# Apokleos/kata-xpu-device-plugin

Measured on NVIDIA H100. Metric: pci.ids parse GB/s (x1000 text + 2^20-key join); device lookups/s reported beside it, higher is better.
Workload: dtype u8

## Files before the change

### kata-xpu-device-plugin_b200/csrc/api.cu

```cuda
#include <algorithm>
#include <cstdlib>
#include <new>
#include <vector>

#include "internal.cuh"
#include "pciids5.cu"
#include "finalize.cuh"
#include "small.cuh"
#include "scan.cuh"

void kx_exchange_destroy(kxpu_ctx *ctx);

static const char *kx_err_names[] = {
    "ok", "invalid argument", "CUDA error", "no sm_90 GPU available", "output buffer too small",
    "table capacity exceeded", "NCCL / peer exchange unavailable or failed", "input outside the supported domain", "out of memory"};

extern "C" const char *kxpu_strerror(int32_t status) {
    int i = -status;
    if (i < 0 || i > 8) return "unknown status";
    return kx_err_names[i];
}

extern "C" const char *kxpu_last_error(kxpu_ctx *ctx) {
    if (!ctx) return "null ctx";
// ... 175 lines not shown
        KX_SET_ERR(ctx, "cudaMalloc(%zu) for the look-back state failed", want * 8);
        return nullptr;
    }
    if (ctx->scan_state) cudaFree(ctx->scan_state);
    ctx->scan_state = p;
    ctx->scan_state_words = want;
    return p;
}

uint32_t kx_next_epoch(kxpu_ctx *ctx) {
    if (++ctx->scan_epoch >= ctx->scan_epoch_limit) {
        if (ctx->scan_state) cudaMemsetAsync(ctx->scan_state, 0, ctx->scan_state_words * 8, ctx->stream);
        ctx->scan_epoch = 1;
    }
    return ctx->scan_epoch;
}

static inline size_t align_up(size_t x, size_t a) { return (x + a - 1) / a * a; }

static inline size_t range_words_bytes(uint32_t num_chunks) { return ((size_t)num_chunks + 64) * 24; }

struct ArenaLayout {
    size_t o_slots, o_vfirst, o_trunc, ff_bytes, o_counters, o_range, o_row_key, o_row_line, o_row_anchor, o_row_noff, o_row_nlen,
        o_sel, o_blob, total;
};
static ArenaLayout arena_layout(uint32_t cap, uint32_t blob_cap, size_t range_bytes) {
    ArenaLayout L;
    const size_t slots = (size_t)cap + 1;
    size_t off = 0;
    L.o_slots = off;       off = align_up(off + slots * sizeof(KxSlot), 256);
    L.o_vfirst = off;      off = align_up(off + 65536 * 8, 256);
    L.o_trunc = off;       off = align_up(off + 8, 256);
    L.ff_bytes = off;
    L.o_counters = off;    off = align_up(off + KX_C_COUNT * 4, 256);
    L.o_range = off;       off = align_up(off + range_bytes, 256);
    L.o_row_key = off;     off = align_up(off + slots * 4, 256);
    L.o_row_line = off;    off = align_up(off + slots * 8, 256);
    L.o_row_anchor = off;  off = align_up(off + slots * 8, 256);
    L.o_row_noff = off;    off = align_up(off + slots * 4, 256);
    L.o_row_nlen = off;    off = align_up(off + slots * 4, 256);
    L.o_sel = off;         off = align_up(off + slots * 4, 256);
    L.o_blob = off;        off = align_up(off + (size_t)blob_cap + 16, 256);
    L.total = off;
    return L;
}

static void arena_reset(kxpu_ctx *ctx, const KxArena &a) {
    const ArenaLayout L = arena_layout(a.cap, a.blob_cap, a.range_bytes);
    const size_t n16 = L.ff_bytes / 16;
    size_t blocks = (n16 + 255) / 256;
    const size_t maxb = (size_t)ctx->sm_count * 8;
    if (blocks > maxb) blocks = maxb;
    kxparse::arena_reset_kernel<<<(unsigned)blocks, 256, 0, ctx->stream>>>((uint4 *)a.p, n16, (uint32_t *)((uint8_t *)a.p + L.o_counters));
    KX_LAUNCHED(ctx);
}

int32_t kx_table_acquire(kxpu_ctx *ctx, uint32_t cap, uint32_t blob_cap, uint32_t num_chunks, kxpu_table **out) {
    kxpu_table *t = new (std::nothrow) kxpu_table();
    if (!t) return KXPU_E_NOMEM;
    const size_t need_range = range_words_bytes(num_chunks);
    bool found = false;
    for (size_t i = 0; i < ctx->pool.size(); i++) {
        const KxArena &a = ctx->pool[i];
        if (a.cap == cap && a.blob_cap == blob_cap && a.range_bytes >= need_range && a.range_bytes <= 4 * need_range + (1u << 20)) {
// ... 22 lines not shown
        }
        arena_reset(ctx, a);
        t->arena = a;
    }
    const ArenaLayout L = arena_layout(cap, blob_cap, t->arena.range_bytes);
    uint8_t *b = (uint8_t *)t->arena.p;
    t->cap = cap;
    uint32_t lg = 0;
    while ((1u << lg) < cap) lg++;
    t->shift = 32 - lg;
    t->dev.slots = (KxSlot *)(b + L.o_slots);
    t->dev.vendor_first = (unsigned long long *)(b + L.o_vfirst);
    t->dev.trunc = (unsigned long long *)(b + L.o_trunc);
    t->dev.counters = (uint32_t *)(b + L.o_counters);
    t->dev.cap = cap;
    t->dev.shift = t->shift;
    t->dev.max_keys = cap / 2;
    t->range_words = (unsigned long long *)(b + L.o_range);
    t->row_key = (uint32_t *)(b + L.o_row_key);
    t->row_line = (unsigned long long *)(b + L.o_row_line);
    t->row_anchor = (unsigned long long *)(b + L.o_row_anchor);
    t->row_name_off = (uint32_t *)(b + L.o_row_noff);
    t->row_name_len = (uint32_t *)(b + L.o_row_nlen);
    t->sel = (uint32_t *)(b + L.o_sel);
    t->blob = b + L.o_blob;
    t->blob_cap = blob_cap;
    t->rows_cap = cap + 1;
    *out = t;
    return KXPU_OK;
}

void kx_table_release(kxpu_ctx *ctx, kxpu_table *t) {
    if (!t) return;
    if (t->arena.p) {
        if (ctx->pool.size() >= 4) {
            cudaStreamSynchronize(ctx->stream);
            cudaFree(ctx->pool.front().p);
            ctx->pool.erase(ctx->pool.begin());
        }
        arena_reset(ctx, t->arena);
        ctx->pool.push_back(t->arena);
    }
    delete t;
}

uint32_t kx_initial_blob_cap(kxpu_ctx *ctx, size_t n) {
    const uint32_t by_text = (uint32_t)std::min<size_t>(std::max<size_t>(n, 256), 4u << 20);
// ... 83 lines not shown
    if (wait) F.wait = *wait;
    F.text = d_text; F.n = n; F.base = base; F.tab = t->dev;
    if (mv) F.mv = *mv;
    else { F.mv.a = t->dev.vendor_first; F.mv.stride = 0; F.mv.n = 1; F.mv.trunc1 = t->dev.trunc; }
    F.row_key = t->row_key; F.row_line = t->row_line; F.row_anchor = t->row_anchor;
    F.row_name_off = t->row_name_off; F.row_name_len = t->row_name_len;
    F.blob = t->blob; F.blob_cap = t->blob_cap;
    if (slab) {
        F.slab_rows = reinterpret_cast<kxx::SlabRow *>(slab->rows); F.slab_rows_cap = slab->rows_cap;
        F.blob = slab->blob; F.blob_cap = slab->blob_cap;
        F.tail = slab->tail;
    }
    KxTimer tm(ctx, KXPU_T_FINALIZE);
    F.scan_w = t->cap >= (1u << 19) ? 32u : 8u;
    if (ctx->force_scan_w) F.scan_w = (uint32_t)ctx->force_scan_w;
    const unsigned batches = (t->cap + 1 + F.scan_w - 1) / F.scan_w;
    const unsigned grid = std::min<unsigned>((batches + kxparse::SF_WARPS - 1) / kxparse::SF_WARPS, 8u * ctx->sm_count);
    kxparse::select_finalize_kernel<<<grid, kxparse::SF_WARPS * 32, 0, ctx->stream>>>(F);
    KX_LAUNCHED(ctx);
    KX_CUDA(ctx, cudaGetLastError());
    return KXPU_OK;
}

int32_t kx_launch_lookup(kxpu_ctx *ctx, kxpu_table *t, const uint32_t *d_keys, size_t n, int32_t *d_rows) {
    if (n == 0) return KXPU_OK;
    KxTimer tm(ctx, KXPU_T_LOOKUP);
    size_t blocks = (n + 255) / 256;
    size_t maxb = (size_t)ctx->sm_count * 32;
    if (blocks > maxb) blocks = maxb;
    kxparse::lookup_kernel<<<(unsigned)blocks, 256, 0, ctx->stream>>>(d_keys, n, t->dev.slots, t->cap, t->shift, d_rows);
    KX_LAUNCHED(ctx);
    KX_CUDA(ctx, cudaGetLastError());
    return KXPU_OK;
}

struct KxJoin {
    const uint32_t *d_keys;
    size_t n;
    int32_t *d_rows;
    int32_t *h_rows;
    const uint8_t *src_text;
};

static void *kx_mapped_host(const void *p) {
    if (!p) return nullptr;
    cudaPointerAttributes at;
    if (cudaPointerGetAttributes(&at, p) != cudaSuccess) { cudaGetLastError(); return nullptr; }
    return at.type == cudaMemoryTypeHost ? at.devicePointer : nullptr;
}

static uint32_t small_text_chunks(kxpu_ctx *ctx) {
    if (ctx->small_chunks < 0) {
        int coop = 0, per_sm = 0;
// ... 89 lines not shown

static int32_t kx_build_table_join(kxpu_ctx *ctx, const uint8_t *d_text, size_t n, kxpu_table **out, const KxJoin *join) {
    if ((reinterpret_cast<uintptr_t>(d_text) & 15u) != 0) {
        KX_SET_ERR(ctx, "device text pointer must be 16-byte aligned");
        return KXPU_E_INVALID;
    }
    if (n >= (1ull << 44)) return KXPU_E_UNSUPPORTED;
    uint32_t cap = ctx->cap_hint;
    while (cap > (1u << 16) && (size_t)cap / 2 > n / 6 + 1) cap >>= 1;
    uint32_t blob_cap = kx_initial_blob_cap(ctx, n);
    const uint32_t num_chunks = (uint32_t)((n + kxparse::CW - 1) / kxparse::CW);
    bool have_trunc = false;
    for (int attempt = 0; attempt < 12; attempt++) {
        kxpu_table *t = nullptr;
        int32_t rc = kx_table_acquire(ctx, cap, blob_cap, num_chunks, &t);
        if (rc != KXPU_OK) return rc;
        const bool small_path = num_chunks > 0 && num_chunks <= small_text_chunks(ctx) && !have_trunc;
        if (small_path) {
            rc = launch_small(ctx, t, d_text, n, join);
        } else {
            if (join && join->src_text && attempt == 0) cudaMemcpyAsync(const_cast<uint8_t *>(d_text), join->src_text, n, cudaMemcpyDefault, ctx->stream);
            rc = kx_launch_parse(ctx, t, d_text, n, 0, 0, nullptr);
            if (rc == KXPU_OK && have_trunc) rc = kx_launch_trunc(ctx, t, d_text, n, 0);
            if (rc == KXPU_OK) rc = kx_launch_finalize(ctx, t, d_text, n, 0, nullptr, nullptr, nullptr);
            if (rc == KXPU_OK && join) rc = kx_launch_lookup(ctx, t, join->d_keys, join->n, join->d_rows);
        }
        if (rc != KXPU_OK) { kx_table_release(ctx, t); return rc; }
        const bool zero_copy = small_path && join && join->src_text;
        if (!zero_copy) {
            if (join && join->h_rows && join->n) cudaMemcpyAsync(join->h_rows, join->d_rows, join->n * 4, cudaMemcpyDeviceToHost, ctx->stream);
            cudaMemcpyAsync(ctx->h_ctl, t->dev.counters, KX_C_COUNT * 4, cudaMemcpyDeviceToHost, ctx->stream);
        }
        cudaError_t e = cudaStreamSynchronize(ctx->stream);
        if (e != cudaSuccess) {
            KX_SET_ERR(ctx, "parse/finalize failed: %s", cudaGetErrorString(e));
            kx_table_release(ctx, t);
            return KXPU_E_CUDA;
        }
        const uint32_t *h = ctx->h_ctl;
        if (h[KX_C_OVERFLOW] || h[KX_C_NKEYS] > t->dev.max_keys) {
            kx_table_release(ctx, t);
            if (!kx_grow_cap(&cap, h[KX_C_OVERFLOW] != 0)) return KXPU_E_CAPACITY;
            continue;
        }
        if (h[KX_C_NEED_TRUNC] == 2u) {
            kx_table_release(ctx, t);
            have_trunc = true;
            continue;
// ... 203 lines not shown
```

### kata-xpu-device-plugin_b200/csrc/finalize.cuh

```cuda
#pragma once
#include "exchange.cuh"
#include "parse_common.cuh"

namespace kxparse {

constexpr unsigned long long MAX_TOKEN = 65536ull;

__global__ void __launch_bounds__(1024) trunc_kernel(const uint8_t *__restrict__ text, unsigned long long n,
                                                      unsigned long long base, unsigned long long *trunc_out, uint32_t *counters) {
    __shared__ unsigned long long s_first[1024], s_last[1024], s_bad[1024];
    const unsigned long long per = (n + 1023ull) / 1024ull;
    const unsigned long long lo = per * threadIdx.x, hi = lo + per < n ? lo + per : n;
    unsigned long long first = KX_NO_OFF, last = KX_NO_OFF, bad = KX_NO_OFF;
    for (unsigned long long i = lo; i < hi; i++) {
        if (text[i] == (uint8_t)'\n') {
            if (first == KX_NO_OFF) first = i;
            else if (i - last - 1 >= MAX_TOKEN && bad == KX_NO_OFF) bad = last + 1;
            last = i;
        }
    }
    s_first[threadIdx.x] = first; s_last[threadIdx.x] = last; s_bad[threadIdx.x] = bad;
    __syncthreads();
    if (threadIdx.x == 0) {
        unsigned long long prev_nl = KX_NO_OFF;
// ... 83 lines not shown
__device__ __forceinline__ void finalize_store_row(const FinalizeParams &F, uint32_t row, uint32_t slot, uint32_t key, unsigned long long line,
                                                   unsigned long long anchor, uint32_t name_off, uint32_t name_len) {
    F.tab.slots[slot].row = (int32_t)row;
    if (F.slab_rows) {
        if (row < F.slab_rows_cap) {
            kxx::SlabRow r;
            r.key = key; r.name_len = name_len; r.line = line; r.anchor = anchor; r.name_off = name_off; r.pad = 0u;
            F.slab_rows[row] = r;
        }
    } else {
        F.row_key[row] = key; F.row_line[row] = line; F.row_anchor[row] = anchor;
        F.row_name_off[row] = name_off; F.row_name_len[row] = name_len;
    }
}

struct SfEntry {
    unsigned long long line, anchor;
    uint32_t slot, key;
};
constexpr int SF_QCAP = SF_BATCH - 1 + 32;

#define SF_MARK(k) do { if (F.trace && threadIdx.x == 0 && F.trace[blockIdx.x * 8u + (k)] == 0) F.trace[blockIdx.x * 8u + (k)] = clock64(); } while (0)

__device__ __forceinline__ void select_finalize_body(const FinalizeParams &F, const uint32_t scan_w) {
    __shared__ __align__(16) uint8_t s_raw[SF_WARPS][4][SF_WIN + 16];
    __shared__ uint8_t s_name[SF_WARPS][SF_BATCH][SF_WIN];
    __shared__ __align__(8) SfEntry s_q[SF_WARPS][SF_QCAP + 1];
    __shared__ uint32_t s_cnt[SF_WARPS], s_bytes[SF_WARPS], s_more[SF_WARPS], s_row0, s_blob0;
    if (F.tab.counters[KX_C_LONGLINE_HINT] != 0u && F.tab.counters[KX_C_NEED_TRUNC] != 1u) {
        if (blockIdx.x == 0 && threadIdx.x == 0) F.tab.counters[KX_C_NEED_TRUNC] = 2u;
        return;
    }
    const uint32_t lane = threadIdx.x & 31u, wl = threadIdx.x >> 5, sub = lane & 7u, grp = lane >> 3;
    const uint32_t nslots = F.tab.cap + 1u;
    const uint32_t nchunks = (nslots + scan_w - 1u) / scan_w;
    const uint32_t cstride = gridDim.x * (uint32_t)SF_WARPS;
    const unsigned long long trunc = kxx::min_view_trunc(F.mv);
    SfEntry *q = s_q[wl];
    uint32_t chunk = blockIdx.x * (uint32_t)SF_WARPS + wl;
    uint32_t qn = 0;
    for (;;) {
        while (qn < (uint32_t)SF_BATCH && chunk < nchunks) {
            const uint32_t slot = chunk * scan_w + lane;
            chunk += cstride;
            bool valid = false;
            uint32_t key = 0;
            unsigned long long line = 0, anchor = 0;
            if (lane < scan_w && slot < nslots) {
                const uint4 head = *reinterpret_cast<const uint4 *>(&F.tab.slots[slot]);
                anchor = F.tab.slots[slot].min_anchor;
                line = ((unsigned long long)head.w << 32) | head.z;
                key = slot == F.tab.cap ? KX_EMPTY_KEY : head.x;
                valid = line != KX_NO_OFF && !(slot < F.tab.cap && key == KX_EMPTY_KEY);
                if (valid) {
                    const unsigned long long a0 = (line - F.base + 5ull) & ~15ull;
                    if (a0 < F.n) asm volatile("prefetch.global.L2 [%0];" ::"l"(F.text + a0));
                    if (a0 + 112ull < F.n && ((a0 + 112ull) >> 7) != (a0 >> 7)) asm volatile("prefetch.global.L2 [%0];" ::"l"(F.text + a0 + 112ull));
                    valid = anchor == kxx::min_view_first(F.mv, key >> 16) && line < trunc;
                }
            }
            const uint32_t vm = __ballot_sync(0xffffffffu, valid);
            if (valid) {
                SfEntry e;
                e.line = line; e.anchor = anchor; e.slot = slot; e.key = key;
                q[qn + (uint32_t)__popc(vm & ((1u << lane) - 1u))] = e;
            }
            qn += (uint32_t)__popc(vm);
            __syncwarp();
        }
        SF_MARK(0);
        const bool have = chunk < nchunks;
        const uint32_t nvalid = qn >= (uint32_t)SF_BATCH ? (uint32_t)SF_BATCH : (have ? 0u : qn);
        uint32_t my_len = 0;
        uint32_t slow_m = 0;
        for (uint32_t r0 = 0; r0 < nvalid; r0 += 4u) {
            const uint32_t r = r0 + grp;
            const bool act = r < nvalid;
            const uint32_t gmask = 0xffu << (8u * grp);
            uint32_t total = 0, start = 0, end = 0;
            bool slow = false;
            const uint8_t *buf = s_raw[wl][grp];
            if (act) {
                const unsigned long long rs = q[r].line - F.base + 5ull;
                const unsigned long long a0 = rs & ~15ull;
                const uint32_t lead = (uint32_t)(rs - a0);
                const unsigned long long p0 = a0 + 16ull * sub;
                uint4 qd;
                if (p0 + 16ull <= F.n) {
                    qd = *reinterpret_cast<const uint4 *>(F.text + p0);
                } else {
                    uint8_t tmp[16];
#pragma unroll
                    for (int k = 0; k < 16; k++) tmp[k] = p0 + k < F.n ? F.text[p0 + k] : (uint8_t)0x0a;
                    qd = *reinterpret_cast<uint4 *>(tmp);
                }
                uint8_t *raw = s_raw[wl][grp];
                *reinterpret_cast<uint4 *>(raw + 16u * sub) = qd;
                uint32_t nlm = 0;
                {
                    const uint32_t w4[4] = {qd.x, qd.y, qd.z, qd.w};
#pragma unroll
                    for (int k = 0; k < 4; k++) {
                        const uint32_t y = w4[k] ^ 0x0a0a0a0au;
                        const uint32_t z = ~(((y & 0x7f7f7f7fu) + 0x7f7f7f7fu) | y | 0x7f7f7f7fu);
                        nlm |= (((z >> 7) * 0x00204081u) >> 21 & 0xfu) << (4 * k);
                    }
                    if (sub == 0u) nlm &= 0xffffu << lead;
                }
                const uint32_t pos = nlm ? (uint32_t)__ffs((int)nlm) - 1u : 16u;
                uint32_t first = pos < 16u ? 16u * sub + pos : (uint32_t)SF_WIN;
#pragma unroll
                for (int d = 4; d > 0; d >>= 1) {
                    const uint32_t o = __shfl_xor_sync(gmask, first, d, 8);
                    first = o < first ? o : first;
                }
                __syncwarp(gmask);
                if (first >= (uint32_t)SF_WIN) {
                    slow = true;
                } else {
                    buf = raw + lead;
                    uint32_t len = first - lead;
                    if (len > 0 && buf[len - 1] == 0x0du) len--;
                    if (sub == 0) trim_space(buf, len, start, end);
                    start = __shfl_sync(gmask, start, 0, 8);
                    end = __shfl_sync(gmask, end, 0, 8);
                }
            }
            {
                const uint32_t span = __reduce_max_sync(0xffffffffu, end - start);
                uint8_t *dst = s_name[wl][act ? r : 0u];
                for (uint32_t o = 0; o < span; o += 8u) {
                    const uint32_t i = start + o + sub;
                    const bool in = i < end;
                    const uint32_t c = in ? buf[i] : 0x41u;
                    const uint32_t prev = (in && i > start) ? buf[i - 1] : 0x41u;
                    const uint32_t nx = (in && i + 1u < end) ? buf[i + 1] : 0u;
                    const bool sp = c <= 32u && ((0x100003600ull >> c) & 1ull);
                    const bool psp = prev <= 32u && ((0x100003600ull >> prev) & 1ull);
                    uint32_t ch = 0;
                    ch = (c - 0x61u < 26u) ? c - 32u : ch;
                    ch = (c - 0x41u < 26u || c - 0x30u < 10u || c == 0x5fu) ? c : ch;
                    ch = (c == 0x2fu || c == 0x2eu) ? 0x5fu : ch;
                    ch = sp ? (psp ? 0u : 0x5fu) : ch;
                    ch = (c == 0xC4u && nx == 0xB1u) ? 0x49u : ch;
                    ch = (c == 0xC5u && nx == 0xBFu) ? 0x53u : ch;
                    ch = in ? ch : 0u;
                    const uint32_t gm = (__ballot_sync(0xffffffffu, ch != 0u) >> (8u * grp)) & 0xffu;
                    if (ch) dst[total + (uint32_t)__popc(gm & ((1u << sub) - 1u))] = (uint8_t)ch;
                    total += (uint32_t)__popc(gm);
                }
            }
            const uint32_t gtot = __shfl_sync(0xffffffffu, total, (lane & 3u) * 8u);
            const uint32_t gslow = __ballot_sync(0xffffffffu, slow && sub == 0u);
            if (lane >= r0 && lane < r0 + 4u && lane < nvalid) my_len = gtot;
            for (uint32_t g = 0; g < 4u; g++)
                if ((gslow >> (8u * g)) & 1u) slow_m |= 1u << (r0 + g);
            __syncwarp();
        }
        __syncwarp();
        SF_MARK(1);
        uint32_t len_r = (lane < nvalid && !((slow_m >> lane) & 1u)) ? my_len : 0u;
        uint32_t incl = len_r;
#pragma unroll
        for (int d = 1; d < 32; d <<= 1) {
            const uint32_t y = __shfl_up_sync(0xffffffffu, incl, d);
            if (lane >= (uint32_t)d) incl += y;
        }
        const uint32_t wtot = __shfl_sync(0xffffffffu, incl, 31);
        if (lane == 0) { s_cnt[wl] = nvalid; s_bytes[wl] = wtot; s_more[wl] = (have || qn > nvalid) ? 1u : 0u; }
        __syncthreads();
        if (threadIdx.x == 0) {
            uint32_t rows = 0, bytes = 0;
#pragma unroll
            for (int k = 0; k < SF_WARPS; k++) { rows += s_cnt[k]; bytes += s_bytes[k]; }
            s_row0 = rows ? atomicAdd(&F.tab.counters[KX_C_NSEL], rows) : 0u;
            uint32_t b0 = bytes ? atomicAdd(&F.tab.counters[KX_C_BLOB_CURSOR], bytes) : 0u;
            if (b0 + bytes > F.blob_cap) { F.tab.counters[KX_C_BLOB_OVERFLOW] = 1u; b0 = 0xFFFFFFFFu; }
            s_blob0 = b0;
        }
        SF_MARK(2);
        __syncthreads();
        SF_MARK(3);
        uint32_t row0 = s_row0, blob0 = s_blob0, more = 0;
        for (uint32_t k = 0; k < wl; k++) { row0 += s_cnt[k]; if (blob0 != 0xFFFFFFFFu) blob0 += s_bytes[k]; }
#pragma unroll
        for (int k = 0; k < SF_WARPS; k++) more |= s_more[k];
        const bool room = blob0 != 0xFFFFFFFFu;
        const uint32_t off_r = room ? blob0 + incl - len_r : 0u;
        for (uint32_t r = 0; r < nvalid; r++) {
            const uint32_t L = __shfl_sync(0xffffffffu, len_r, r), O = __shfl_sync(0xffffffffu, off_r, r);
            if (room)
                for (uint32_t j = lane; j < L; j += 32u) F.blob[O + j] = s_name[wl][r][j];
        }
        if (lane < nvalid && !((slow_m >> lane) & 1u)) {
            const SfEntry e = q[lane];
            finalize_store_row(F, row0 + lane, e.slot, e.key, e.line, e.anchor, room ? off_r : 0u, room ? len_r : 0u);
        }
        SF_MARK(4);
        __syncwarp();
        for (uint32_t sm = slow_m; sm; sm &= sm - 1u) {
            const uint32_t r = (uint32_t)__ffs((int)sm) - 1u;
            const unsigned long long l_line = q[r].line, l_anchor = q[r].anchor;
            const uint32_t l_key = q[r].key, l_slot = q[r].slot;
            const unsigned long long rs = l_line - F.base + 5ull;
            uint8_t *buf = &s_name[wl][0][0];
            constexpr uint32_t LONG_MAX_LEN = (uint32_t)(SF_BATCH * SF_WIN) - 32u;
            uint32_t len = 0;
            bool found = false;
            for (uint32_t o = 0; o < LONG_MAX_LEN + 32u && !found; o += 32u) {
                const unsigned long long pos = rs + o + lane;
                const uint32_t c = pos < F.n ? F.text[pos] : 0x0au;
                buf[o + lane] = (uint8_t)c;
                const uint32_t nlm = __ballot_sync(0xffffffffu, c == 0x0au);
                if (nlm) { len = o + (uint32_t)__ffs((int)nlm) - 1u; found = true; }
            }
            __syncwarp();
            uint32_t start = 0, end = 0, out_len = 0, at = 0;
            bool ok = true;
            if (found) {
                if (len > 0 && buf[len - 1] == 0x0du) len--;
                if (lane == 0) trim_space(buf, len, start, end);
                start = __shfl_sync(0xffffffffu, start, 0);
                end = __shfl_sync(0xffffffffu, end, 0);
                for (uint32_t o = start; o < end; o += 32u) {
                    const uint32_t i = o + lane;
                    const uint32_t ch = i < end ? sanitise_byte(buf, i, start, end) : 0u;
                    out_len += (uint32_t)__popc(__ballot_sync(0xffffffffu, ch != 0u));
                }
                if (lane == 0) {
                    at = out_len ? atomicAdd(&F.tab.counters[KX_C_BLOB_CURSOR], out_len) : 0u;
                    if (at + out_len > F.blob_cap) { F.tab.counters[KX_C_BLOB_OVERFLOW] = 1u; at = 0xFFFFFFFFu; }
                }
                at = __shfl_sync(0xffffffffu, at, 0);
                ok = at != 0xFFFFFFFFu;
                if (ok) {
                    uint32_t wr = at;
                    for (uint32_t o = start; o < end; o += 32u) {
                        const uint32_t i = o + lane;
                        const uint32_t ch = i < end ? sanitise_byte(buf, i, start, end) : 0u;
                        const uint32_t bm = __ballot_sync(0xffffffffu, ch != 0u);
                        if (ch) F.blob[wr + (uint32_t)__popc(bm & ((1u << lane) - 1u))] = (uint8_t)ch;
                        wr += (uint32_t)__popc(bm);
                    }
                }
            } else if (lane == 0) {
                const uint8_t *g = F.text + rs;
                const unsigned long long avail = F.n - rs;
                unsigned long long l = 0;
                while (l < avail && g[l] != 0x0au) l++;
                len = (uint32_t)l;
                if (len > 0 && g[len - 1] == 0x0du) len--;
                trim_space(g, len, start, end);
                for (uint32_t i = start; i < end; i++) out_len += sanitise_byte(g, i, start, end) != 0u;
                at = out_len ? atomicAdd(&F.tab.counters[KX_C_BLOB_CURSOR], out_len) : 0u;
                if (at + out_len > F.blob_cap) { F.tab.counters[KX_C_BLOB_OVERFLOW] = 1u; ok = false; }
                if (ok) {
                    uint32_t wr = at;
                    for (uint32_t i = start; i < end; i++) {
                        const uint32_t ch = sanitise_byte(g, i, start, end);
                        if (ch) F.blob[wr++] = (uint8_t)ch;
                    }
                }
            }
            if (lane == 0) finalize_store_row(F, row0 + r, l_slot, l_key, l_line, l_anchor, ok ? at : 0u, ok ? out_len : 0u);
            __syncwarp();
        }
        SF_MARK(5);
        {
            const uint32_t rem = qn - nvalid;
            if (nvalid != 0u && rem != 0u) {
                SfEntry e;
                if (lane < rem) e = q[nvalid + lane];
                __syncwarp();
                if (lane < rem) q[lane] = e;
                __syncwarp();
            }
            qn = rem;
        }
        __syncthreads();
        SF_MARK(6);
        if (!more) break;
    }
}

__global__ void __launch_bounds__(SF_WARPS * 32, 8) select_finalize_kernel(const FinalizeParams F) {
    kxx::wait_flags_cta(F.wait);
    select_finalize_body(F, F.scan_w);
// ... 4 lines not shown
            const uint32_t prev = atomicAdd(F.tail.done, 1u);
            if (prev == gridDim.x - 1u) {
                *F.tail.done = 0u;
                kx_fence_gpu();
                const volatile uint32_t *c = F.tab.counters;
                const uint32_t n_sel = c[KX_C_NSEL], blob_used = c[KX_C_BLOB_CURSOR];
                const bool over = c[KX_C_BLOB_OVERFLOW] || n_sel > F.tail.rows_cap || blob_used > F.tail.blob_cap;
                kxx::SlabHeader h;
                memset(&h, 0, sizeof h);
                h.n_rows = over ? 0u : n_sel;
                h.blob_bytes = over ? 0u : blob_used;
                h.status = over ? kxx::XS_SLAB_OVERFLOW : 0u;
                if (c[KX_C_OVERFLOW]) h.status |= kxx::XS_GROW | kxx::XS_FULL;
                if (c[KX_C_NKEYS] > F.tab.max_keys) h.status |= kxx::XS_GROW;
                h.nkeys = c[KX_C_NKEYS];
                *F.tail.header = h;
                kx_fence_sys();
                for (int k = 0; k < F.tail.tg.n; k++) *reinterpret_cast<volatile uint32_t *>(F.tail.tg.region[k] + F.tail.o_flag) = F.tail.epoch;
            }
        }
    }
}

__global__ void __launch_bounds__(256) lookup_kernel(const uint32_t *__restrict__ keys, size_t n, const KxSlot *__restrict__ slots,
                                                      uint32_t cap, uint32_t shift, int32_t *__restrict__ rows_out) {
    size_t i = (size_t)blockIdx.x * blockDim.x + threadIdx.x;
    const size_t stride = (size_t)gridDim.x * blockDim.x;
    for (; i < n; i += stride) rows_out[i] = table_probe(slots, cap, shift, keys[i]);
}

__global__ void __launch_bounds__(256) name_len_kernel(const int32_t *__restrict__ rows, size_t n,
                                                        const uint32_t *__restrict__ row_name_len, uint32_t n_rows,
                                                        uint32_t *__restrict__ lens) {
    size_t i = (size_t)blockIdx.x * blockDim.x + threadIdx.x;
    if (i < n) {
        int32_t r = rows[i];
        lens[i] = (r >= 0 && (uint32_t)r < n_rows) ? row_name_len[r] : 0u;
    }
}
__global__ void __launch_bounds__(256) name_copy_kernel(const int32_t *__restrict__ rows, size_t n,
                                                         const uint32_t *__restrict__ row_name_off,
                                                         const uint32_t *__restrict__ row_name_len, uint32_t n_rows,
                                                         const uint8_t *__restrict__ blob,
                                                         const uint32_t *__restrict__ offsets, uint8_t *__restrict__ out,
                                                         size_t cap) {
    size_t i = ((size_t)blockIdx.x * blockDim.x + threadIdx.x) >> 3;
// ... 18 lines not shown
```

### kata-xpu-device-plugin_b200/csrc/internal.cuh

```cuda
#pragma once
#include "common.cuh"
#include "exchange.cuh"
#include "table.cuh"

struct kxpu_table {
    uint32_t cap = 0, shift = 0;
    KxArena arena;
    KxTableDev dev{};
    unsigned long long *range_words = nullptr;
    uint32_t *row_key = nullptr;
    unsigned long long *row_line = nullptr;
    unsigned long long *row_anchor = nullptr;
    uint32_t *row_name_off = nullptr;
    uint32_t *row_name_len = nullptr;
    uint32_t *sel = nullptr;
    uint8_t *blob = nullptr;
    uint32_t blob_cap = 0;
    uint32_t rows_cap = 0;
    uint32_t n_rows = 0;
    uint32_t blob_used = 0;
};

#define KX_ENTER(ctx)                          \
    if (!(ctx)) return KXPU_E_INVALID;         \
    std::lock_guard<std::mutex> guard__((ctx)->mu); \
    cudaSetDevice((ctx)->device)

int32_t kx_table_acquire(kxpu_ctx *ctx, uint32_t cap, uint32_t blob_cap, uint32_t num_chunks, kxpu_table **out);
void kx_table_release(kxpu_ctx *ctx, kxpu_table *t);
uint32_t kx_initial_blob_cap(kxpu_ctx *ctx, size_t n);
struct KxXaHook {
    kxx::XaParams p;
    uint32_t *done;
};
int32_t kx_launch_parse(kxpu_ctx *ctx, kxpu_table *t, const uint8_t *d_text, size_t n, unsigned long long base,
                        unsigned long long carry_in, const KxXaHook *xa);
int32_t kx_launch_trunc(kxpu_ctx *ctx, kxpu_table *t, const uint8_t *d_text, size_t n, unsigned long long base);
struct KxSlabOut {
// ... 12 lines not shown
```

Before: 2417.

## Split finalize into row-select and name pass, co-scheduling names with join lookups

Replaces the single select_finalize kernel on the large-text path with two kernels. The first compacts valid slots into rows with one thread per slot and a per-CTA atomic row claim. The second builds and sanitises names in row order while extra CTAs run the key-lookup join concurrently, which removes the separate lookup launch and overlaps the probe traffic with name building. It also drops the unused sel buffer from the arena. In exchange, row order now follows CTA claim order, and lookups read slot rows that the earlier kernel has already written.

```diff
diff --git a/kata-xpu-device-plugin_b200/csrc/api.cu b/kata-xpu-device-plugin_b200/csrc/api.cu
--- a/kata-xpu-device-plugin_b200/csrc/api.cu
+++ b/kata-xpu-device-plugin_b200/csrc/api.cu
@@ -221,7 +221,7 @@
 
 struct ArenaLayout {
     size_t o_slots, o_vfirst, o_trunc, ff_bytes, o_counters, o_range, o_row_key, o_row_line, o_row_anchor, o_row_noff, o_row_nlen,
-        o_sel, o_blob, total;
+        o_blob, total;
 };
 static ArenaLayout arena_layout(uint32_t cap, uint32_t blob_cap, size_t range_bytes) {
     ArenaLayout L;
@@ -238,7 +238,6 @@
     L.o_row_anchor = off;  off = align_up(off + slots * 8, 256);
     L.o_row_noff = off;    off = align_up(off + slots * 4, 256);
     L.o_row_nlen = off;    off = align_up(off + slots * 4, 256);
-    L.o_sel = off;         off = align_up(off + slots * 4, 256);
     L.o_blob = off;        off = align_up(off + (size_t)blob_cap + 16, 256);
     L.total = off;
     return L;
@@ -307,7 +306,6 @@
     t->row_anchor = (unsigned long long *)(b + L.o_row_anchor);
     t->row_name_off = (uint32_t *)(b + L.o_row_noff);
     t->row_name_len = (uint32_t *)(b + L.o_row_nlen);
-    t->sel = (uint32_t *)(b + L.o_sel);
     t->blob = b + L.o_blob;
     t->blob_cap = blob_cap;
     t->rows_cap = cap + 1;
@@ -437,13 +435,34 @@
     return KXPU_OK;
 }
 
+static unsigned join_ctas(kxpu_ctx *ctx, size_t n) { return (unsigned)std::min<size_t>((n + 255) / 256, (size_t)ctx->sm_count * 32); }
+
 int32_t kx_launch_lookup(kxpu_ctx *ctx, kxpu_table *t, const uint32_t *d_keys, size_t n, int32_t *d_rows) {
     if (n == 0) return KXPU_OK;
     KxTimer tm(ctx, KXPU_T_LOOKUP);
-    size_t blocks = (n + 255) / 256;
-    size_t maxb = (size_t)ctx->sm_count * 32;
-    if (blocks > maxb) blocks = maxb;
-    kxparse::lookup_kernel<<<(unsigned)blocks, 256, 0, ctx->stream>>>(d_keys, n, t->dev.slots, t->cap, t->shift, d_rows);
+    kxparse::lookup_kernel<<<join_ctas(ctx, n), 256, 0, ctx->stream>>>(d_keys, n, t->dev.slots, t->cap, t->shift, d_rows);
+    KX_LAUNCHED(ctx);
+    KX_CUDA(ctx, cudaGetLastError());
+    return KXPU_OK;
+}
+
+static int32_t kx_launch_rows_names_join(kxpu_ctx *ctx, kxpu_table *t, const uint8_t *d_text, size_t n, const uint32_t *d_keys,
+                                         size_t nq, int32_t *d_rows) {
+    using namespace kxparse;
+    FinalizeParams F;
+    memset(&F, 0, sizeof F);
+    F.text = d_text; F.n = n; F.base = 0; F.tab = t->dev;
+    F.mv.a = t->dev.vendor_first; F.mv.stride = 0; F.mv.n = 1; F.mv.trunc1 = t->dev.trunc;
+    F.row_key = t->row_key; F.row_line = t->row_line; F.row_anchor = t->row_anchor;
+    F.row_name_off = t->row_name_off; F.row_name_len = t->row_name_len;
+    F.blob = t->blob; F.blob_cap = t->blob_cap;
+    KxTimer tm(ctx, KXPU_T_FINALIZE);
+    select_rows_kernel<<<(t->cap + SF_WARPS * 32) / (SF_WARPS * 32), SF_WARPS * 32, 0, ctx->stream>>>(F);
+    KX_LAUNCHED(ctx);
+    const uint32_t want = (t->cap / 2 + SF_CTA_ROWS - 1) / SF_CTA_ROWS;
+    const unsigned name_ctas = std::max<unsigned>(1u, std::min<unsigned>(want, 8u * ctx->sm_count));
+    const unsigned grid = name_ctas + (nq ? join_ctas(ctx, nq) : 0u);
+    names_join_kernel<<<grid, SF_WARPS * 32, 0, ctx->stream>>>(F, name_ctas, d_keys, nq, d_rows);
     KX_LAUNCHED(ctx);
     KX_CUDA(ctx, cudaGetLastError());
     return KXPU_OK;
@@ -579,8 +598,9 @@
             if (join && join->src_text && attempt == 0) cudaMemcpyAsync(const_cast<uint8_t *>(d_text), join->src_text, n, cudaMemcpyDefault, ctx->stream);
             rc = kx_launch_parse(ctx, t, d_text, n, 0, 0, nullptr);
             if (rc == KXPU_OK && have_trunc) rc = kx_launch_trunc(ctx, t, d_text, n, 0);
-            if (rc == KXPU_OK) rc = kx_launch_finalize(ctx, t, d_text, n, 0, nullptr, nullptr, nullptr);
-            if (rc == KXPU_OK && join) rc = kx_launch_lookup(ctx, t, join->d_keys, join->n, join->d_rows);
+            if (rc == KXPU_OK)
+                rc = join ? kx_launch_rows_names_join(ctx, t, d_text, n, join->d_keys, join->n, join->d_rows)
+                          : kx_launch_rows_names_join(ctx, t, d_text, n, nullptr, 0, nullptr);
         }
         if (rc != KXPU_OK) { kx_table_release(ctx, t); return rc; }
         const bool zero_copy = small_path && join && join->src_text;
diff --git a/kata-xpu-device-plugin_b200/csrc/finalize.cuh b/kata-xpu-device-plugin_b200/csrc/finalize.cuh
--- a/kata-xpu-device-plugin_b200/csrc/finalize.cuh
+++ b/kata-xpu-device-plugin_b200/csrc/finalize.cuh
@@ -129,16 +129,223 @@
 
 #define SF_MARK(k) do { if (F.trace && threadIdx.x == 0 && F.trace[blockIdx.x * 8u + (k)] == 0) F.trace[blockIdx.x * 8u + (k)] = clock64(); } while (0)
 
+__device__ __forceinline__ bool sf_stand_back(const FinalizeParams &F) {
+    if (F.tab.counters[KX_C_LONGLINE_HINT] != 0u && F.tab.counters[KX_C_NEED_TRUNC] != 1u) {
+        if (blockIdx.x == 0 && threadIdx.x == 0) F.tab.counters[KX_C_NEED_TRUNC] = 2u;
+        return true;
+    }
+    return false;
+}
+
+__device__ __forceinline__ bool sf_slot_valid(const FinalizeParams &F, uint32_t slot, unsigned long long trunc, uint32_t &key,
+                                              unsigned long long &line, unsigned long long &anchor) {
+    const uint4 head = *reinterpret_cast<const uint4 *>(&F.tab.slots[slot]);
+    anchor = F.tab.slots[slot].min_anchor;
+    line = ((unsigned long long)head.w << 32) | head.z;
+    key = slot == F.tab.cap ? KX_EMPTY_KEY : head.x;
+    bool valid = line != KX_NO_OFF && !(slot < F.tab.cap && key == KX_EMPTY_KEY);
+    if (valid) {
+        const unsigned long long a0 = (line - F.base + 5ull) & ~15ull;
+        if (a0 < F.n) asm volatile("prefetch.global.L2 [%0];" ::"l"(F.text + a0));
+        if (a0 + 112ull < F.n && ((a0 + 112ull) >> 7) != (a0 >> 7)) asm volatile("prefetch.global.L2 [%0];" ::"l"(F.text + a0 + 112ull));
+        valid = anchor == kxx::min_view_first(F.mv, key >> 16) && line < trunc;
+    }
+    return valid;
+}
+
+__device__ __forceinline__ void sf_cta_claim(const FinalizeParams &F, uint32_t rows, uint32_t bytes, uint32_t &row0, uint32_t &blob0) {
+    row0 = rows ? atomicAdd(&F.tab.counters[KX_C_NSEL], rows) : 0u;
+    uint32_t b0 = bytes ? atomicAdd(&F.tab.counters[KX_C_BLOB_CURSOR], bytes) : 0u;
+    if (b0 + bytes > F.blob_cap) { F.tab.counters[KX_C_BLOB_OVERFLOW] = 1u; b0 = 0xFFFFFFFFu; }
+    blob0 = b0;
+}
+
+__device__ __forceinline__ void sf_name_batch(const FinalizeParams &F, unsigned long long my_line, uint32_t nvalid,
+                                              uint8_t (*raw_w)[SF_WIN + 16], uint8_t (*name_w)[SF_WIN], uint32_t &my_len,
+                                              uint32_t &slow_m) {
+    const uint32_t lane = threadIdx.x & 31u, sub = lane & 7u, grp = lane >> 3;
+    my_len = 0;
+    slow_m = 0;
+    for (uint32_t r0 = 0; r0 < nvalid; r0 += 4u) {
+        const uint32_t r = r0 + grp;
+        const bool act = r < nvalid;
+        const unsigned long long line_r = __shfl_sync(0xffffffffu, my_line, r);
+        const uint32_t gmask = 0xffu << (8u * grp);
+        uint32_t total = 0, start = 0, end = 0;
+        bool slow = false;
+        const uint8_t *buf = raw_w[grp];
+        if (act) {
+            const unsigned long long rs = line_r - F.base + 5ull;
+            const unsigned long long a0 = rs & ~15ull;
+            const uint32_t lead = (uint32_t)(rs - a0);
+            const unsigned long long p0 = a0 + 16ull * sub;
+            uint4 qd;
+            if (p0 + 16ull <= F.n) {
+                qd = *reinterpret_cast<const uint4 *>(F.text + p0);
+            } else {
+                uint8_t tmp[16];
+#pragma unroll
+                for (int k = 0; k < 16; k++) tmp[k] = p0 + k < F.n ? F.text[p0 + k] : (uint8_t)0x0a;
+                qd = *reinterpret_cast<uint4 *>(tmp);
+            }
+            uint8_t *raw = raw_w[grp];
+            *reinterpret_cast<uint4 *>(raw + 16u * sub) = qd;
+            uint32_t nlm = 0;
+            {
+                const uint32_t w4[4] = {qd.x, qd.y, qd.z, qd.w};
+#pragma unroll
+                for (int k = 0; k < 4; k++) {
+                    const uint32_t y = w4[k] ^ 0x0a0a0a0au;
+                    const uint32_t z = ~(((y & 0x7f7f7f7fu) + 0x7f7f7f7fu) | y | 0x7f7f7f7fu);
+                    nlm |= (((z >> 7) * 0x00204081u) >> 21 & 0xfu) << (4 * k);
+                }
+                if (sub == 0u) nlm &= 0xffffu << lead;
+            }
+            const uint32_t pos = nlm ? (uint32_t)__ffs((int)nlm) - 1u : 16u;
+            uint32_t first = pos < 16u ? 16u * sub + pos : (uint32_t)SF_WIN;
+#pragma unroll
+            for (int d = 4; d > 0; d >>= 1) {
+                const uint32_t o = __shfl_xor_sync(gmask, first, d, 8);
+                first = o < first ? o : first;
+            }
+            __syncwarp(gmask);
+            if (first >= (uint32_t)SF_WIN) {
+                slow = true;
+            } else {
+                buf = raw + lead;
+                uint32_t len = first - lead;
+                if (len > 0 && buf[len - 1] == 0x0du) len--;
+                if (sub == 0) trim_space(buf, len, start, end);
+                start = __shfl_sync(gmask, start, 0, 8);
+                end = __shfl_sync(gmask, end, 0, 8);
+            }
+        }
+        {
+            const uint32_t span = __reduce_max_sync(0xffffffffu, end - start);
+            uint8_t *dst = name_w[act ? r : 0u];
+            for (uint32_t o = 0; o < span; o += 8u) {
+                const uint32_t i = start + o + sub;
+                const bool in = i < end;
+                const uint32_t c = in ? buf[i] : 0x41u;
+                const uint32_t prev = (in && i > start) ? buf[i - 1] : 0x41u;
+                const uint32_t nx = (in && i + 1u < end) ? buf[i + 1] : 0u;
+                const bool sp = c <= 32u && ((0x100003600ull >> c) & 1ull);
+                const bool psp = prev <= 32u && ((0x100003600ull >> prev) & 1ull);
+                uint32_t ch = 0;
+                ch = (c - 0x61u < 26u) ? c - 32u : ch;
+                ch = (c - 0x41u < 26u || c - 0x30u < 10u || c == 0x5fu) ? c : ch;
+                ch = (c == 0x2fu || c == 0x2eu) ? 0x5fu : ch;
+                ch = sp ? (psp ? 0u : 0x5fu) : ch;
+                ch = (c == 0xC4u && nx == 0xB1u) ? 0x49u : ch;
+                ch = (c == 0xC5u && nx == 0xBFu) ? 0x53u : ch;
+                ch = in ? ch : 0u;
+                const uint32_t gm = (__ballot_sync(0xffffffffu, ch != 0u) >> (8u * grp)) & 0xffu;
+                if (ch) dst[total + (uint32_t)__popc(gm & ((1u << sub) - 1u))] = (uint8_t)ch;
+                total += (uint32_t)__popc(gm);
+            }
+        }
+        const uint32_t gtot = __shfl_sync(0xffffffffu, total, (lane & 3u) * 8u);
+        const uint32_t gslow = __ballot_sync(0xffffffffu, slow && sub == 0u);
+        if (lane >= r0 && lane < r0 + 4u && lane < nvalid) my_len = gtot;
+        for (uint32_t g = 0; g < 4u; g++)
+            if ((gslow >> (8u * g)) & 1u) slow_m |= 1u << (r0 + g);
+        __syncwarp();
+    }
+    __syncwarp();
+}
+
+__device__ __forceinline__ uint32_t sf_incl_scan(uint32_t x) {
+    const uint32_t lane = threadIdx.x & 31u;
+#pragma unroll
+    for (int d = 1; d < 32; d <<= 1) {
+        const uint32_t y = __shfl_up_sync(0xffffffffu, x, d);
+        if (lane >= (uint32_t)d) x += y;
+    }
+    return x;
+}
+
+__device__ __forceinline__ void sf_names_out(const FinalizeParams &F, const uint8_t (*name_w)[SF_WIN], uint32_t nvalid, uint32_t len_r,
+                                             uint32_t off_r) {
+    const uint32_t lane = threadIdx.x & 31u;
+    for (uint32_t r = 0; r < nvalid; r++) {
+        const uint32_t L = __shfl_sync(0xffffffffu, len_r, r), O = __shfl_sync(0xffffffffu, off_r, r);
+        for (uint32_t j = lane; j < L; j += 32u) F.blob[O + j] = name_w[r][j];
+    }
+}
+
+__device__ __forceinline__ void sf_long_name(const FinalizeParams &F, unsigned long long line, uint8_t *buf, uint32_t &name_off,
+                                             uint32_t &name_len) {
+    const uint32_t lane = threadIdx.x & 31u;
+    const unsigned long long rs = line - F.base + 5ull;
+    constexpr uint32_t LONG_MAX_LEN = (uint32_t)(SF_BATCH * SF_WIN) - 32u;
+    uint32_t len = 0;
+    bool found = false;
+    for (uint32_t o = 0; o < LONG_MAX_LEN + 32u && !found; o += 32u) {
+        const unsigned long long pos = rs + o + lane;
+        const uint32_t c = pos < F.n ? F.text[pos] : 0x0au;
+        buf[o + lane] = (uint8_t)c;
+        const uint32_t nlm = __ballot_sync(0xffffffffu, c == 0x0au);
+        if (nlm) { len = o + (uint32_t)__ffs((int)nlm) - 1u; found = true; }
+    }
+    __syncwarp();
+    uint32_t start = 0, end = 0, out_len = 0, at = 0;
+    bool ok = true;
+    if (found) {
+        if (len > 0 && buf[len - 1] == 0x0du) len--;
+        if (lane == 0) trim_space(buf, len, start, end);
+        start = __shfl_sync(0xffffffffu, start, 0);
+        end = __shfl_sync(0xffffffffu, end, 0);
+        for (uint32_t o = start; o < end; o += 32u) {
+            const uint32_t i = o + lane;
+            const uint32_t ch = i < end ? sanitise_byte(buf, i, start, end) : 0u;
+            out_len += (uint32_t)__popc(__ballot_sync(0xffffffffu, ch != 0u));
+        }
+        if (lane == 0) {
+            at = out_len ? atomicAdd(&F.tab.counters[KX_C_BLOB_CURSOR], out_len) : 0u;
+            if (at + out_len > F.blob_cap) { F.tab.counters[KX_C_BLOB_OVERFLOW] = 1u; at = 0xFFFFFFFFu; }
+        }
+        at = __shfl_sync(0xffffffffu, at, 0);
+        ok = at != 0xFFFFFFFFu;
+        if (ok) {
+            uint32_t wr = at;
+            for (uint32_t o = start; o < end; o += 32u) {
+                const uint32_t i = o + lane;
+                const uint32_t ch = i < end ? sanitise_byte(buf, i, start, end) : 0u;
+                const uint32_t bm = __ballot_sync(0xffffffffu, ch != 0u);
+                if (ch) F.blob[wr + (uint32_t)__popc(bm & ((1u << lane) - 1u))] = (uint8_t)ch;
+                wr += (uint32_t)__popc(bm);
+            }
+        }
+    } else if (lane == 0) {
+        const uint8_t *g = F.text + rs;
+        const unsigned long long avail = F.n - rs;
+        unsigned long long l = 0;
+        while (l < avail && g[l] != 0x0au) l++;
+        len = (uint32_t)l;
+        if (len > 0 && g[len - 1] == 0x0du) len--;
+        trim_space(g, len, start, end);
+        for (uint32_t i = start; i < end; i++) out_len += sanitise_byte(g, i, start, end) != 0u;
+        at = out_len ? atomicAdd(&F.tab.counters[KX_C_BLOB_CURSOR], out_len) : 0u;
+        if (at + out_len > F.blob_cap) { F.tab.counters[KX_C_BLOB_OVERFLOW] = 1u; ok = false; }
+        if (ok) {
+            uint32_t wr = at;
+            for (uint32_t i = start; i < end; i++) {
+                const uint32_t ch = sanitise_byte(g, i, start, end);
+                if (ch) F.blob[wr++] = (uint8_t)ch;
+            }
+        }
+    }
+    name_off = ok ? at : 0u;
+    name_len = ok ? out_len : 0u;
+}
+
 __device__ __forceinline__ void select_finalize_body(const FinalizeParams &F, const uint32_t scan_w) {
     __shared__ __align__(16) uint8_t s_raw[SF_WARPS][4][SF_WIN + 16];
     __shared__ uint8_t s_name[SF_WARPS][SF_BATCH][SF_WIN];
     __shared__ __align__(8) SfEntry s_q[SF_WARPS][SF_QCAP + 1];
     __shared__ uint32_t s_cnt[SF_WARPS], s_bytes[SF_WARPS], s_more[SF_WARPS], s_row0, s_blob0;
-    if (F.tab.counters[KX_C_LONGLINE_HINT] != 0u && F.tab.counters[KX_C_NEED_TRUNC] != 1u) {
-        if (blockIdx.x == 0 && threadIdx.x == 0) F.tab.counters[KX_C_NEED_TRUNC] = 2u;
-        return;
-    }
-    const uint32_t lane = threadIdx.x & 31u, wl = threadIdx.x >> 5, sub = lane & 7u, grp = lane >> 3;
+    if (sf_stand_back(F)) return;
+    const uint32_t lane = threadIdx.x & 31u, wl = threadIdx.x >> 5;
     const uint32_t nslots = F.tab.cap + 1u;
     const uint32_t nchunks = (nslots + scan_w - 1u) / scan_w;
     const uint32_t cstride = gridDim.x * (uint32_t)SF_WARPS;
@@ -150,22 +357,9 @@
         while (qn < (uint32_t)SF_BATCH && chunk < nchunks) {
             const uint32_t slot = chunk * scan_w + lane;
             chunk += cstride;
-            bool valid = false;
             uint32_t key = 0;
             unsigned long long line = 0, anchor = 0;
-            if (lane < scan_w && slot < nslots) {
-                const uint4 head = *reinterpret_cast<const uint4 *>(&F.tab.slots[slot]);
-                anchor = F.tab.slots[slot].min_anchor;
-                line = ((unsigned long long)head.w << 32) | head.z;
-                key = slot == F.tab.cap ? KX_EMPTY_KEY : head.x;
-                valid = line != KX_NO_OFF && !(slot < F.tab.cap && key == KX_EMPTY_KEY);
-                if (valid) {
-                    const unsigned long long a0 = (line - F.base + 5ull) & ~15ull;
-                    if (a0 < F.n) asm volatile("prefetch.global.L2 [%0];" ::"l"(F.text + a0));
-                    if (a0 + 112ull < F.n && ((a0 + 112ull) >> 7) != (a0 >> 7)) asm volatile("prefetch.global.L2 [%0];" ::"l"(F.text + a0 + 112ull));
-                    valid = anchor == kxx::min_view_first(F.mv, key >> 16) && line < trunc;
-                }
-            }
+            const bool valid = lane < scan_w && slot < nslots && sf_slot_valid(F, slot, trunc, key, line, anchor);
             const uint32_t vm = __ballot_sync(0xffffffffu, valid);
             if (valid) {
                 SfEntry e;
@@ -178,101 +372,11 @@
         SF_MARK(0);
         const bool have = chunk < nchunks;
         const uint32_t nvalid = qn >= (uint32_t)SF_BATCH ? (uint32_t)SF_BATCH : (have ? 0u : qn);
-        uint32_t my_len = 0;
-        uint32_t slow_m = 0;
-        for (uint32_t r0 = 0; r0 < nvalid; r0 += 4u) {
-            const uint32_t r = r0 + grp;
-            const bool act = r < nvalid;
-            const uint32_t gmask = 0xffu << (8u * grp);
-            uint32_t total = 0, start = 0, end = 0;
-            bool slow = false;
-            const uint8_t *buf = s_raw[wl][grp];
-            if (act) {
-                const unsigned long long rs = q[r].line - F.base + 5ull;
-                const unsigned long long a0 = rs & ~15ull;
-                const uint32_t lead = (uint32_t)(rs - a0);
-                const unsigned long long p0 = a0 + 16ull * sub;
-                uint4 qd;
-                if (p0 + 16ull <= F.n) {
-                    qd = *reinterpret_cast<const uint4 *>(F.text + p0);
-                } else {
-                    uint8_t tmp[16];
-#pragma unroll
-                    for (int k = 0; k < 16; k++) tmp[k] = p0 + k < F.n ? F.text[p0 + k] : (uint8_t)0x0a;
-                    qd = *reinterpret_cast<uint4 *>(tmp);
-                }
-                uint8_t *raw = s_raw[wl][grp];
-                *reinterpret_cast<uint4 *>(raw + 16u * sub) = qd;
-                uint32_t nlm = 0;
-                {
-                    const uint32_t w4[4] = {qd.x, qd.y, qd.z, qd.w};
-#pragma unroll
-                    for (int k = 0; k < 4; k++) {
-                        const uint32_t y = w4[k] ^ 0x0a0a0a0au;
-                        const uint32_t z = ~(((y & 0x7f7f7f7fu) + 0x7f7f7f7fu) | y | 0x7f7f7f7fu);
-                        nlm |= (((z >> 7) * 0x00204081u) >> 21 & 0xfu) << (4 * k);
-                    }
-                    if (sub == 0u) nlm &= 0xffffu << lead;
-                }
-                const uint32_t pos = nlm ? (uint32_t)__ffs((int)nlm) - 1u : 16u;
-                uint32_t first = pos < 16u ? 16u * sub + pos : (uint32_t)SF_WIN;
-#pragma unroll
-                for (int d = 4; d > 0; d >>= 1) {
-                    const uint32_t o = __shfl_xor_sync(gmask, first, d, 8);
-                    first = o < first ? o : first;
-                }
-                __syncwarp(gmask);
-                if (first >= (uint32_t)SF_WIN) {
-                    slow = true;
-                } else {
-                    buf = raw + lead;
-                    uint32_t len = first - lead;
-                    if (len > 0 && buf[len - 1] == 0x0du) len--;
-                    if (sub == 0) trim_space(buf, len, start, end);
-                    start = __shfl_sync(gmask, start, 0, 8);
-                    end = __shfl_sync(gmask, end, 0, 8);
-                }
-            }
-            {
-                const uint32_t span = __reduce_max_sync(0xffffffffu, end - start);
-                uint8_t *dst = s_name[wl][act ? r : 0u];
-                for (uint32_t o = 0; o < span; o += 8u) {
-                    const uint32_t i = start + o + sub;
-                    const bool in = i < end;
-                    const uint32_t c = in ? buf[i] : 0x41u;
-                    const uint32_t prev = (in && i > start) ? buf[i - 1] : 0x41u;
-                    const uint32_t nx = (in && i + 1u < end) ? buf[i + 1] : 0u;
-                    const bool sp = c <= 32u && ((0x100003600ull >> c) & 1ull);
-                    const bool psp = prev <= 32u && ((0x100003600ull >> prev) & 1ull);
-                    uint32_t ch = 0;
-                    ch = (c - 0x61u < 26u) ? c - 32u : ch;
-                    ch = (c - 0x41u < 26u || c - 0x30u < 10u || c == 0x5fu) ? c : ch;
-                    ch = (c == 0x2fu || c == 0x2eu) ? 0x5fu : ch;
-                    ch = sp ? (psp ? 0u : 0x5fu) : ch;
-                    ch = (c == 0xC4u && nx == 0xB1u) ? 0x49u : ch;
-                    ch = (c == 0xC5u && nx == 0xBFu) ? 0x53u : ch;
-                    ch = in ? ch : 0u;
-                    const uint32_t gm = (__ballot_sync(0xffffffffu, ch != 0u) >> (8u * grp)) & 0xffu;
-                    if (ch) dst[total + (uint32_t)__popc(gm & ((1u << sub) - 1u))] = (uint8_t)ch;
-                    total += (uint32_t)__popc(gm);
-                }
-            }
-            const uint32_t gtot = __shfl_sync(0xffffffffu, total, (lane & 3u) * 8u);
-            const uint32_t gslow = __ballot_sync(0xffffffffu, slow && sub == 0u);
-            if (lane >= r0 && lane < r0 + 4u && lane < nvalid) my_len = gtot;
-            for (uint32_t g = 0; g < 4u; g++)
-                if ((gslow >> (8u * g)) & 1u) slow_m |= 1u << (r0 + g);
-            __syncwarp();
-        }
-        __syncwarp();
+        uint32_t my_len, slow_m;
+        sf_name_batch(F, lane < nvalid ? q[lane].line : 0ull, nvalid, s_raw[wl], s_name[wl], my_len, slow_m);
         SF_MARK(1);
-        uint32_t len_r = (lane < nvalid && !((slow_m >> lane) & 1u)) ? my_len : 0u;
-        uint32_t incl = len_r;
-#pragma unroll
-        for (int d = 1; d < 32; d <<= 1) {
-            const uint32_t y = __shfl_up_sync(0xffffffffu, incl, d);
-            if (lane >= (uint32_t)d) incl += y;
-        }
+        const uint32_t len_r = (lane < nvalid && !((slow_m >> lane) & 1u)) ? my_len : 0u;
+        const uint32_t incl = sf_incl_scan(len_r);
         const uint32_t wtot = __shfl_sync(0xffffffffu, incl, 31);
         if (lane == 0) { s_cnt[wl] = nvalid; s_bytes[wl] = wtot; s_more[wl] = (have || qn > nvalid) ? 1u : 0u; }
         __syncthreads();
@@ -280,10 +384,7 @@
             uint32_t rows = 0, bytes = 0;
 #pragma unroll
             for (int k = 0; k < SF_WARPS; k++) { rows += s_cnt[k]; bytes += s_bytes[k]; }
-            s_row0 = rows ? atomicAdd(&F.tab.counters[KX_C_NSEL], rows) : 0u;
-            uint32_t b0 = bytes ? atomicAdd(&F.tab.counters[KX_C_BLOB_CURSOR], bytes) : 0u;
-            if (b0 + bytes > F.blob_cap) { F.tab.counters[KX_C_BLOB_OVERFLOW] = 1u; b0 = 0xFFFFFFFFu; }
-            s_blob0 = b0;
+            sf_cta_claim(F, rows, bytes, s_row0, s_blob0);
         }
         SF_MARK(2);
         __syncthreads();
@@ -293,83 +394,20 @@
 #pragma unroll
         for (int k = 0; k < SF_WARPS; k++) more |= s_more[k];
         const bool room = blob0 != 0xFFFFFFFFu;
-        const uint32_t off_r = room ? blob0 + incl - len_r : 0u;
-        for (uint32_t r = 0; r < nvalid; r++) {
-            const uint32_t L = __shfl_sync(0xffffffffu, len_r, r), O = __shfl_sync(0xffffffffu, off_r, r);
-            if (room)
-                for (uint32_t j = lane; j < L; j += 32u) F.blob[O + j] = s_name[wl][r][j];
-        }
+        const uint32_t off_r = room ? blob0 + incl - len_r : 0u, len_w = room ? len_r : 0u;
+        sf_names_out(F, s_name[wl], nvalid, len_w, off_r);
         if (lane < nvalid && !((slow_m >> lane) & 1u)) {
             const SfEntry e = q[lane];
-            finalize_store_row(F, row0 + lane, e.slot, e.key, e.line, e.anchor, room ? off_r : 0u, room ? len_r : 0u);
+            finalize_store_row(F, row0 + lane, e.slot, e.key, e.line, e.anchor, off_r, len_w);
         }
         SF_MARK(4);
         __syncwarp();
         for (uint32_t sm = slow_m; sm; sm &= sm - 1u) {
             const uint32_t r = (uint32_t)__ffs((int)sm) - 1u;
-            const unsigned long long l_line = q[r].line, l_anchor = q[r].anchor;
-            const uint32_t l_key = q[r].key, l_slot = q[r].slot;
-            const unsigned long long rs = l_line - F.base + 5ull;
-            uint8_t *buf = &s_name[wl][0][0];
-            constexpr uint32_t LONG_MAX_LEN = (uint32_t)(SF_BATCH * SF_WIN) - 32u;
-            uint32_t len = 0;
-            bool found = false;
-            for (uint32_t o = 0; o < LONG_MAX_LEN + 32u && !found; o += 32u) {
-                const unsigned long long pos = rs + o + lane;
-                const uint32_t c = pos < F.n ? F.text[pos] : 0x0au;
-                buf[o + lane] = (uint8_t)c;
-                const uint32_t nlm = __ballot_sync(0xffffffffu, c == 0x0au);
-                if (nlm) { len = o + (uint32_t)__ffs((int)nlm) - 1u; found = true; }
-            }
-            __syncwarp();
-            uint32_t start = 0, end = 0, out_len = 0, at = 0;
-            bool ok = true;
-            if (found) {
-                if (len > 0 && buf[len - 1] == 0x0du) len--;
-                if (lane == 0) trim_space(buf, len, start, end);
-                start = __shfl_sync(0xffffffffu, start, 0);
-                end = __shfl_sync(0xffffffffu, end, 0);
-                for (uint32_t o = start; o < end; o += 32u) {
-                    const uint32_t i = o + lane;
-                    const uint32_t ch = i < end ? sanitise_byte(buf, i, start, end) : 0u;
-                    out_len += (uint32_t)__popc(__ballot_sync(0xffffffffu, ch != 0u));
-                }
-                if (lane == 0) {
-                    at = out_len ? atomicAdd(&F.tab.counters[KX_C_BLOB_CURSOR], out_len) : 0u;
-                    if (at + out_len > F.blob_cap) { F.tab.counters[KX_C_BLOB_OVERFLOW] = 1u; at = 0xFFFFFFFFu; }
-                }
-                at = __shfl_sync(0xffffffffu, at, 0);
-                ok = at != 0xFFFFFFFFu;
-                if (ok) {
-                    uint32_t wr = at;
-                    for (uint32_t o = start; o < end; o += 32u) {
-                        const uint32_t i = o + lane;
-                        const uint32_t ch = i < end ? sanitise_byte(buf, i, start, end) : 0u;
-                        const uint32_t bm = __ballot_sync(0xffffffffu, ch != 0u);
-                        if (ch) F.blob[wr + (uint32_t)__popc(bm & ((1u << lane) - 1u))] = (uint8_t)ch;
-                        wr += (uint32_t)__popc(bm);
-                    }
-                }
-            } else if (lane == 0) {
-                const uint8_t *g = F.text + rs;
-                const unsigned long long avail = F.n - rs;
-                unsigned long long l = 0;
-                while (l < avail && g[l] != 0x0au) l++;
-                len = (uint32_t)l;
-                if (len > 0 && g[len - 1] == 0x0du) len--;
-                trim_space(g, len, start, end);
-                for (uint32_t i = start; i < end; i++) out_len += sanitise_byte(g, i, start, end) != 0u;
-                at = out_len ? atomicAdd(&F.tab.counters[KX_C_BLOB_CURSOR], out_len) : 0u;
-                if (at + out_len > F.blob_cap) { F.tab.counters[KX_C_BLOB_OVERFLOW] = 1u; ok = false; }
-                if (ok) {
-                    uint32_t wr = at;
-                    for (uint32_t i = start; i < end; i++) {
-                        const uint32_t ch = sanitise_byte(g, i, start, end);
-                        if (ch) F.blob[wr++] = (uint8_t)ch;
-                    }
-                }
-            }
-            if (lane == 0) finalize_store_row(F, row0 + r, l_slot, l_key, l_line, l_anchor, ok ? at : 0u, ok ? out_len : 0u);
+            const SfEntry e = q[r];
+            uint32_t name_off, name_len;
+            sf_long_name(F, e.line, &s_name[wl][0][0], name_off, name_len);
+            if (lane == 0) finalize_store_row(F, row0 + r, e.slot, e.key, e.line, e.anchor, name_off, name_len);
             __syncwarp();
         }
         SF_MARK(5);
@@ -420,6 +458,87 @@
     }
 }
 
+constexpr uint32_t SF_CTA_ROWS = SF_WARPS * SF_BATCH;
+
+__global__ void __launch_bounds__(SF_WARPS * 32) select_rows_kernel(const FinalizeParams F) {
+    __shared__ uint32_t s_cnt[SF_WARPS], s_row0;
+    if (sf_stand_back(F)) return;
+    const uint32_t lane = threadIdx.x & 31u, wl = threadIdx.x >> 5;
+    const uint32_t slot = blockIdx.x * blockDim.x + threadIdx.x;
+    uint32_t key = 0;
+    unsigned long long line = 0, anchor = 0;
+    const bool valid = slot <= F.tab.cap && sf_slot_valid(F, slot, kxx::min_view_trunc(F.mv), key, line, anchor);
+    const uint32_t vm = __ballot_sync(0xffffffffu, valid);
+    if (lane == 0) s_cnt[wl] = (uint32_t)__popc(vm);
+    __syncthreads();
+    if (threadIdx.x == 0) {
+        uint32_t rows = 0, blob0;
+#pragma unroll
+        for (int k = 0; k < SF_WARPS; k++) rows += s_cnt[k];
+        sf_cta_claim(F, rows, 0u, s_row0, blob0);
+    }
+    __syncthreads();
+    if (valid) {
+        uint32_t row = s_row0 + (uint32_t)__popc(vm & ((1u << lane) - 1u));
+        for (uint32_t k = 0; k < wl; k++) row += s_cnt[k];
+        F.tab.slots[slot].row = (int32_t)row;
+        F.row_key[row] = key; F.row_line[row] = line; F.row_anchor[row] = anchor;
+    }
+}
+
+__device__ __forceinline__ void names_body(const FinalizeParams &F, uint32_t ctas) {
+    __shared__ __align__(16) uint8_t s_raw[SF_WARPS][4][SF_WIN + 16];
+    __shared__ uint8_t s_name[SF_WARPS][SF_BATCH][SF_WIN];
+    __shared__ uint32_t s_bytes[SF_WARPS], s_blob0;
+    const uint32_t lane = threadIdx.x & 31u, wl = threadIdx.x >> 5;
+    const uint32_t n_rows = F.tab.counters[KX_C_NSEL];
+    for (uint32_t c0 = blockIdx.x * SF_CTA_ROWS; c0 < n_rows; c0 += ctas * SF_CTA_ROWS) {
+        const uint32_t r0 = c0 + wl * (uint32_t)SF_BATCH;
+        const uint32_t nvalid = r0 < n_rows ? min(n_rows - r0, (uint32_t)SF_BATCH) : 0u;
+        uint32_t my_len, slow_m;
+        sf_name_batch(F, lane < nvalid ? F.row_line[r0 + lane] : 0ull, nvalid, s_raw[wl], s_name[wl], my_len, slow_m);
+        const uint32_t len_r = (lane < nvalid && !((slow_m >> lane) & 1u)) ? my_len : 0u;
+        const uint32_t incl = sf_incl_scan(len_r);
+        const uint32_t wtot = __shfl_sync(0xffffffffu, incl, 31);
+        if (lane == 0) s_bytes[wl] = wtot;
+        __syncthreads();
+        if (threadIdx.x == 0) {
+            uint32_t bytes = 0, row0;
+#pragma unroll
+            for (int k = 0; k < SF_WARPS; k++) bytes += s_bytes[k];
+            sf_cta_claim(F, 0u, bytes, row0, s_blob0);
+        }
+        __syncthreads();
+        uint32_t blob0 = s_blob0;
+        for (uint32_t k = 0; k < wl; k++) if (blob0 != 0xFFFFFFFFu) blob0 += s_bytes[k];
+        const bool room = blob0 != 0xFFFFFFFFu;
+        const uint32_t off_r = room ? blob0 + incl - len_r : 0u, len_w = room ? len_r : 0u;
+        sf_names_out(F, s_name[wl], nvalid, len_w, off_r);
+        if (lane < nvalid && !((slow_m >> lane) & 1u)) { F.row_name_off[r0 + lane] = off_r; F.row_name_len[r0 + lane] = len_w; }
+        __syncwarp();
+        for (uint32_t sm = slow_m; sm; sm &= sm - 1u) {
+            const uint32_t r = (uint32_t)__ffs((int)sm) - 1u;
+            uint32_t name_off, name_len;
+            sf_long_name(F, F.row_line[r0 + r], &s_name[wl][0][0], name_off, name_len);
+            if (lane == 0) { F.row_name_off[r0 + r] = name_off; F.row_name_len[r0 + r] = name_len; }
+            __syncwarp();
+        }
+        __syncthreads();
+    }
+}
+
+__global__ void __launch_bounds__(SF_WARPS * 32, 8) names_join_kernel(const FinalizeParams F, uint32_t name_ctas,
+                                                                       const uint32_t *__restrict__ keys, size_t nq,
+                                                                       int32_t *__restrict__ rows_out) {
+    if (blockIdx.x < name_ctas) {
+        names_body(F, name_ctas);
+        return;
+    }
+    const size_t stride = (size_t)(gridDim.x - name_ctas) * blockDim.x;
+    for (size_t i = (size_t)(blockIdx.x - name_ctas) * blockDim.x + threadIdx.x; i < nq; i += stride)
+        rows_out[i] = table_probe(F.tab.slots, F.tab.cap, F.tab.shift, keys[i]);
+}
+
 __global__ void __launch_bounds__(256) lookup_kernel(const uint32_t *__restrict__ keys, size_t n, const KxSlot *__restrict__ slots,
                                                       uint32_t cap, uint32_t shift, int32_t *__restrict__ rows_out) {
     size_t i = (size_t)blockIdx.x * blockDim.x + threadIdx.x;
diff --git a/kata-xpu-device-plugin_b200/csrc/internal.cuh b/kata-xpu-device-plugin_b200/csrc/internal.cuh
--- a/kata-xpu-device-plugin_b200/csrc/internal.cuh
+++ b/kata-xpu-device-plugin_b200/csrc/internal.cuh
@@ -13,7 +13,6 @@
     unsigned long long *row_anchor = nullptr;
     uint32_t *row_name_off = nullptr;
     uint32_t *row_name_len = nullptr;
-    uint32_t *sel = nullptr;
     uint8_t *blob = nullptr;
     uint32_t blob_cap = 0;
     uint32_t rows_cap = 0;
```

New measurement: 2516, median of 6. 1.04x the previous value.
